# re-ovo/wgpu-path-tracing

Measured on AMD Instinct MI355X. Metric: Msamples/s (rays x bounces / s), higher is better.
Workload: dtype f32

## Files before the change

### wgpu-path-tracing_amd/csrc/pt_device.h

```cpp
#pragma once
#include <hip/hip_runtime.h>
#include <stdint.h>
#include <initializer_list>
#include <variant>
#include "ptmi_layout.h"
#include "ptmi.h"

#define PT_HD __host__ __device__ inline

#define PT_REF_LEAF      0x80000000u
#define PT_REF_NONE      0xFFFFFFFFu
#define PT_LEAF_MAX_TRIS 32u
#define PT_LEAF_OFF_BITS 26u
#define PT_LEAF_OFF_MASK ((1u << PT_LEAF_OFF_BITS) - 1u)

struct DevEnv {
    const float4 *tab;
    const uint2 *alias;
    uint32_t w, h;
    uint32_t sampled;
    float intensity, rotation;
};

struct DevMedium {
// ... 136 lines not shown
              "ptmi_reproject zeroes the four with one memset, ptmi_reproject_status reads them with one copy");
static_assert(kCtRpMoved == kCtRpSamples + 1 && kCtRpMovedCarried == kCtRpMoved + 1,
              "the two motion words follow the four: the same memset zeroes all six, ptmi_motion_status reads the two with one copy");

struct ShadeParams {
    uint32_t bounce, max_bounces, do_mis;
    uint32_t *counts;
    uint32_t emit_records;
    const uint32_t *pid;
};

enum { PT_VARIANT_GLOBAL = 1, PT_VARIANT_LDS = 2, PT_VARIANT_LDS_NODES = 3,
       PT_VARIANT_OWN_LDS = 4, PT_VARIANT_OWN_LDS_NODES = 5, PT_VARIANT_OWN_QLDS = 6, PT_VARIANT_OWN_QLDS_NODES = 7,
       PT_VARIANT_OWN_QGLOBAL = 8, PT_VARIANT_OWN_GLOBAL = 9,
       PT_VARIANT_OWN_LDS16_NODES = 10,
       PT_VARIANT_OWN_QLDS16_NODES = 11,
       PT_VARIANT_COUNT };

enum PtNodes {
    PT_NODES_EXACT,
    PT_NODES_QUANT,
    PT_NODES_EXACT16,
    PT_NODES_QUANT16 };
enum PtWhere {
    PT_LDS_ALL,
    PT_LDS_NODES,
    PT_FROM_MEMORY };
enum PtStack {
    PT_STACK_DEPTH,
    PT_STACK_NODES,
    PT_STACK_SPILL,
    PT_STACK_16BIT,
    PT_STACK_16BIT_SPILL };
struct PtVariant { PtNodes nodes; PtWhere where; PtStack stack; bool own; };
constexpr PtVariant kPtVariants[PT_VARIANT_COUNT] = {
    {},
    {PT_NODES_EXACT,   PT_FROM_MEMORY, PT_STACK_SPILL,       false},
    {PT_NODES_EXACT,   PT_LDS_ALL,     PT_STACK_DEPTH,       false},
    {PT_NODES_EXACT,   PT_LDS_NODES,   PT_STACK_NODES,       false},
    {PT_NODES_EXACT,   PT_LDS_ALL,     PT_STACK_DEPTH,       true},
    {PT_NODES_EXACT,   PT_LDS_NODES,   PT_STACK_NODES,       true},
    {PT_NODES_QUANT,   PT_LDS_ALL,     PT_STACK_DEPTH,       true},
    {PT_NODES_QUANT,   PT_LDS_NODES,   PT_STACK_NODES,       true},
    {PT_NODES_QUANT,   PT_FROM_MEMORY, PT_STACK_SPILL,       true},
    {PT_NODES_EXACT,   PT_FROM_MEMORY, PT_STACK_SPILL,       true},
    {PT_NODES_EXACT16, PT_LDS_NODES,   PT_STACK_16BIT,       true},
    {PT_NODES_QUANT16, PT_LDS_NODES,   PT_STACK_16BIT_SPILL, true},
};
inline const PtVariant &pt_variant(int v) { return kPtVariants[v > 0 && v < PT_VARIANT_COUNT ? v : 0]; }
inline bool pt_quantised(const PtVariant &r) { return r.nodes == PT_NODES_QUANT || r.nodes == PT_NODES_QUANT16; }
inline bool pt_spills(const PtVariant &r, int wgs) {
    return r.stack == PT_STACK_SPILL || r.stack == PT_STACK_16BIT_SPILL || (r.stack == PT_STACK_NODES && wgs == 1);
}
inline size_t pt_lds_bytes(const PtVariant &r, uint32_t n_nodes, uint32_t n_tris, int entries) {
    if (r.where == PT_FROM_MEMORY) return 0;
    const bool narrow = r.nodes == PT_NODES_EXACT16 || r.nodes == PT_NODES_QUANT16;
    return (size_t)n_nodes * (pt_quantised(r) ? 32 : 64) + (r.where == PT_LDS_ALL ? (size_t)n_tris * 48 : 0) +
           (size_t)entries * 1024 * (narrow ? sizeof(uint16_t) : sizeof(uint32_t));
}

struct TraverseConfig {
    int variant;
    int stack_entries;
    int cull;
    int wgs_per_cu;
    size_t lds_bytes;
    uint32_t *spill;
    int wants_spill;
    int quantized;
};
inline uint32_t pt_variant_code(const TraverseConfig &cfg) { return (uint32_t)cfg.variant * 10u + (uint32_t)cfg.wgs_per_cu; }
#ifndef PT_QCACHE_NODES
#define PT_QCACHE_NODES 256
#endif
#define PT_SPILL_ENTRIES 64
size_t pt_spill_bytes(int blocks);

struct DensePixels {
    DevBand band; uint32_t frame0;
    __device__ uint32_t entries() const { return band.rows * band.width; }
    __device__ uint32_t pixel(uint32_t j) const { return j; }
    __device__ uint32_t first_frame(size_t) const { return frame0; }
    __device__ void count_paths(uint32_t) const {}
};
struct ListedPixels {
    DevBand band; const uint32_t *list, *n_active; const float4 *mom;
    unsigned long long *traced;
    __device__ uint32_t entries() const { return *n_active; }
    __device__ uint32_t pixel(uint32_t j) const { return list[j]; }
    __device__ uint32_t first_frame(size_t oi) const { return (uint32_t)mom[oi].z; }
    __device__ void count_paths(uint32_t paths) const { atomicAdd(traced, (unsigned long long)paths); }
};
struct BakedPixels {
    DevBand band; const uint32_t *covered; uint32_t n, frame0;
    __device__ uint32_t entries() const { return n; }
    __device__ uint32_t pixel(uint32_t j) const { return covered[j]; }
    __device__ uint32_t first_frame(size_t) const { return frame0; }
    __device__ void count_paths(uint32_t) const {}
};
using DevPixels = std::variant<DensePixels, ListedPixels, BakedPixels>;
struct CameraSource { const ptmi_camera *cam; uint32_t proj; };
struct BakeSurface { const float4 *texels; float bias; };
struct ProbeSet { const float4 *probes; uint32_t shift, cols, count; };
using DevRays = std::variant<CameraSource, BakeSurface, ProbeSet>;
void pt_launch_raygen(hipStream_t s, int blocks, const DevRays &rays, const DevPixels &px, uint32_t n_frames, DevPaths p, uint32_t *count_out);
void pt_launch_raygen_list(hipStream_t s, const DevRays &rays, uint32_t width, uint32_t n, const uint32_t *xs, const uint32_t *ys,
                           const uint32_t *frames, DevPaths p);
float4 *pt_launch_bake_dilate(hipStream_t s, uint32_t W, uint32_t H, uint32_t passes, const float4 *texels, const float4 *out,
                              float4 *a, float4 *b);
struct DevProbeAtlas { const float4 *out; const float4 *probes; uint32_t W, shift, cols, count; };
// ... 108 lines not shown
```

### wgpu-path-tracing_amd/csrc/traverse.hip

```cpp
#include "pt_device.h"
#include "pt_math.h"
#include "traverse_common.h"

namespace {

struct GlobalMem {
    glb_f4p wn, tp;
    PT_DEV void node(uint32_t i, bool, Boxes &o) const { float4 a, b, c, r; load_node(wn + 4u * (size_t)i, a, b, c, r); boxes_of(a, b, c, r, o); }
    PT_DEV bool open(uint32_t ref, bool, v3, v3, float, uint32_t &first, uint32_t &cnt, uint32_t &cursor) const {
        open_plain(ref, first, cnt, cursor); return true;
    }
    PT_DEV void tri(uint32_t cursor, uint32_t k, bool, float4 &a, float4 &b, float4 &c) const {
        glb_f4p p = tp + 3u * (size_t)(cursor + k);
        a = as_f4(p[0]); b = as_f4(p[1]); c = as_f4(p[2]);
    }
};
template <bool TRIS_IN_LDS>
struct LdsMem {
    lds_f4p wn, tl; glb_f4p tg;
    PT_DEV void node(uint32_t i, bool, Boxes &o) const {
        lds_f4p p = wn + 4u * i;
        boxes_of(as_f4(p[0]), as_f4(p[1]), as_f4(p[2]), as_f4(p[3]), o);
    }
    PT_DEV bool open(uint32_t ref, bool, v3, v3, float, uint32_t &first, uint32_t &cnt, uint32_t &cursor) const {
        open_plain(ref, first, cnt, cursor); return true;
    }
    PT_DEV void tri(uint32_t cursor, uint32_t k, bool, float4 &a, float4 &b, float4 &c) const {
        const uint32_t i = cursor + k;
        if (TRIS_IN_LDS) { lds_f4p p = tl + 3u * i; a = as_f4(p[0]); b = as_f4(p[1]); c = as_f4(p[2]); }
        else { glb_f4p p = tg + 3u * (size_t)i; a = as_f4(p[0]); b = as_f4(p[1]); c = as_f4(p[2]); }
    }
};

typedef const __attribute__((address_space(1))) uint32_t *glb_u32p;
typedef uint32_t u4v __attribute__((ext_vector_type(4)));
typedef const __attribute__((address_space(1))) u4v *glb_u4p;
typedef const __attribute__((address_space(3))) u4v *lds_u4p;
struct QuantMem {
    glb_u4p qn; glb_u32p ls; glb_f4p tp;
    float ox, oy, oz, sx, sy, sz;
    lds_u4p qc; uint32_t n_cached;
    PT_DEV void node(uint32_t i, bool, Boxes &b) const {
        u4v l, r;
        if (i < n_cached) { l = qc[2u * i]; r = qc[2u * i + 1u]; }
        else { l = qn[2u * (size_t)i]; r = qn[2u * (size_t)i + 1u]; }
        b.lx0 = fma1(sx, (float)(l.x & 0xFFFFu), ox); b.ly0 = fma1(sy, (float)(l.x >> 16), oy);
        b.lz0 = fma1(sz, (float)(l.y & 0xFFFFu), oz); b.lx1 = fma1(sx, (float)(l.y >> 16), ox);
        b.ly1 = fma1(sy, (float)(l.z & 0xFFFFu), oy); b.lz1 = fma1(sz, (float)(l.z >> 16), oz);
        b.rx0 = fma1(sx, (float)(r.x & 0xFFFFu), ox); b.ry0 = fma1(sy, (float)(r.x >> 16), oy);
        b.rz0 = fma1(sz, (float)(r.y & 0xFFFFu), oz); b.rx1 = fma1(sx, (float)(r.y >> 16), ox);
        b.ry1 = fma1(sy, (float)(r.z & 0xFFFFu), oy); b.rz1 = fma1(sz, (float)(r.z >> 16), oz);
        b.lref = l.w; b.rref = r.w;
    }
    PT_DEV bool open(uint32_t ref, bool plain, v3 o, v3 inv, float limit, uint32_t &first, uint32_t &cnt, uint32_t &cursor) const {
        if (plain) { open_plain(ref, first, cnt, cursor); return true; }
        const uint32_t off = ref & ~PT_REF_LEAF;
        glb_u32p h = ls + off;
        const float lx = __uint_as_float(h[0]), ly = __uint_as_float(h[1]), lz = __uint_as_float(h[2]);
        first = h[3];
        const float hx = __uint_as_float(h[4]), hy = __uint_as_float(h[5]), hz = __uint_as_float(h[6]);
        cnt = h[7];
        cursor = off + 8u;
        float tl;
        const bool pass = slab(lx, ly, lz, hx, hy, hz, o, inv, tl);
        return pass & !(tl > limit);
    }
    PT_DEV void tri(uint32_t cursor, uint32_t k, bool plain, float4 &a, float4 &b, float4 &c) const {
        if (plain) {
            glb_f4p p = tp + 3u * (size_t)(cursor + k);
            a = as_f4(p[0]); b = as_f4(p[1]); c = as_f4(p[2]);
        } else {
            glb_u32p p = ls + cursor + 9u * k;
            a = make_float4(__uint_as_float(p[0]), __uint_as_float(p[1]), __uint_as_float(p[2]), 0.0f);
            b = make_float4(__uint_as_float(p[3]), __uint_as_float(p[4]), __uint_as_float(p[5]), 0.0f);
            c = make_float4(__uint_as_float(p[6]), __uint_as_float(p[7]), __uint_as_float(p[8]), 0.0f);
// ... 149 lines not shown
                    cn = cn & (cur != PT_REF_NONE) & ((int)room2(lp, sp, stride) | (int)(SPILL && (sp != bot) & room2(lp, bot, stride)));
                    if (popc(ballot(cn)) * NODE_KEEP < popc(bn)) break;
                }
            }
        }
        };
        if (ballot(slow & active) != 0ull) streams(std::true_type{});
        else streams(std::false_type{});
        const bool stuck = active & !can_node & !can_tri & ((bn | bt) == 0ull);
        const bool done = active & (occluded | stuck | ((cur == PT_REF_NONE) & (lp == top)));
        if (done) { io.finish(slot, best, occluded); active = false; cur = PT_REF_NONE; lp = top; }
    }
#ifdef PT_UTIL_STATS
    if (lane == 0u) for (int i = 0; i < 8; i++) atomicAdd(&g_util[MODE][i], (unsigned long long)ut[i]);
    for (int i = 8; i < 10; i++) if (ut[i]) atomicAdd(&g_util[MODE][i], (unsigned long long)ut[i]);
#endif
}

constexpr int GBLOCK = 256;

template <int MODE, bool CULL, int STACK, bool QUANT, class IO>
__global__ __launch_bounds__(GBLOCK) void k_trace_global(DevScene sc, IO io, const uint32_t *__restrict__ count_ptr,
                                                         uint32_t *__restrict__ spill) {
    __shared__ uint32_t stk[STACK * GBLOCK];
    const uint32_t count = *count_ptr;
    const uint32_t gw = (threadIdx.x >> 6) * gridDim.x + blockIdx.x;
    uint32_t *sp = spill + (size_t)blockIdx.x * GBLOCK + threadIdx.x;
    if constexpr (QUANT) {
        __shared__ uint4 qcache[2 * PT_QCACHE_NODES];
        const uint32_t nc = sc.q_cached < PT_QCACHE_NODES ? sc.q_cached : PT_QCACHE_NODES;
        if (blockIdx.x * 64u >= count) return;
        for (uint32_t i = threadIdx.x; i < 2u * nc; i += GBLOCK) qcache[i] = sc.qnodes[i];
        __syncthreads();
        if (gw * 64u >= count) return;
        QuantMem m{(glb_u4p)sc.qnodes, (glb_u32p)sc.leaf_stream, (glb_f4p)sc.tripos,
                   sc.q_origin[0], sc.q_origin[1], sc.q_origin[2], sc.q_scale[0], sc.q_scale[1], sc.q_scale[2],
                   (lds_u4p)qcache, nc};
        trace_wave<MODE, CULL, STACK, true, PT_REFILL_GLOBAL>(m, sc, io, count, gw, gridDim.x * (GBLOCK / 64), stk + threadIdx.x, GBLOCK, sp, gridDim.x * GBLOCK);
    } else {
        if (gw * 64u >= count) return;
        GlobalMem m{(glb_f4p)sc.wnodes, (glb_f4p)sc.tripos};
        trace_wave<MODE, CULL, STACK, true, PT_REFILL_GLOBAL>(m, sc, io, count, gw, gridDim.x * (GBLOCK / 64), stk + threadIdx.x, GBLOCK, sp, gridDim.x * GBLOCK);
    }
}

constexpr int LBLOCK = 1024;

template <int MODE, bool CULL, int STACK, bool TRIS_IN_LDS, bool SPILL, class IO>
__global__ __launch_bounds__(LBLOCK) void k_trace_lds(DevScene sc, IO io, const uint32_t *__restrict__ count_ptr,
                                                      uint32_t *__restrict__ spill) {
    extern __shared__ float4 smem[];
    const uint32_t count = *count_ptr;
    if (blockIdx.x * 64u >= count) return;
    const uint32_t nw = 4u * sc.n_wnodes, nt = TRIS_IN_LDS ? 3u * sc.n_tris : 0u;
    for (uint32_t i = threadIdx.x; i < nw; i += LBLOCK) smem[i] = sc.wnodes[i];
    for (uint32_t i = threadIdx.x; i < nt; i += LBLOCK) smem[nw + i] = sc.tripos[i];
    __syncthreads();
    const uint32_t gw = (threadIdx.x >> 6) * gridDim.x + blockIdx.x;
    if (gw * 64u >= count) return;
    LdsMem<TRIS_IN_LDS> m{(lds_f4p)smem, (lds_f4p)(smem + nw), (glb_f4p)sc.tripos};
    uint32_t *stk = reinterpret_cast<uint32_t *>(smem + nw + nt) + threadIdx.x;
    trace_wave<MODE, CULL, STACK, SPILL, REFILL_AT>(m, sc, io, count, gw, gridDim.x * (LBLOCK / 64), stk, LBLOCK,
                                           SPILL ? spill + (size_t)blockIdx.x * LBLOCK + threadIdx.x : nullptr, gridDim.x * LBLOCK);
}

template <int MODE, bool CULL, int STACK, bool TRIS, bool SPILL, class IO>
void launch_lds(hipStream_t s, int wgs, const TraverseConfig &cfg, const DevScene &sc, const IO &io, const uint32_t *count) {
    allow_all_lds<k_trace_lds<MODE, CULL, STACK, TRIS, SPILL, IO>>();
    hipLaunchKernelGGL((k_trace_lds<MODE, CULL, STACK, TRIS, SPILL, IO>), dim3(wgs), dim3(LBLOCK), cfg.lds_bytes, s, sc, io, count,
                       SPILL ? cfg.spill : nullptr);
}
template <int MODE, bool CULL, bool QUANT, class IO>
void launch_global(hipStream_t s, int cus, const DevScene &sc, const IO &io, const uint32_t *count, uint32_t *spill) {
    const int per_cu = resident_wgs_per_cu<k_trace_global<MODE, CULL, 16, QUANT, IO>>(GBLOCK);
    hipLaunchKernelGGL((k_trace_global<MODE, CULL, 16, QUANT, IO>), dim3(per_cu * cus), dim3(GBLOCK), 0, s, sc, io, count, spill);
}

template <int MODE, bool CULL, class IO>
void launch(hipStream_t s, int blocks, const TraverseConfig &cfg, const DevScene &sc, const IO &io, const uint32_t *count) {
    const int cus = blocks / 8 > 0 ? blocks / 8 : 1;
    const int wgs = cfg.wgs_per_cu * cus;
    if (cfg.variant == PT_VARIANT_LDS_NODES && cfg.wgs_per_cu == 1) {
        launch_lds<MODE, CULL, 16, false, true>(s, wgs, cfg, sc, io, count);
    } else if (cfg.variant == PT_VARIANT_LDS_NODES) {
        if (cfg.stack_entries <= 15) launch_lds<MODE, CULL, 15, false, false>(s, wgs, cfg, sc, io, count);
        else launch_lds<MODE, CULL, 16, false, false>(s, wgs, cfg, sc, io, count);
    } else if (cfg.variant == PT_VARIANT_LDS) {
        if (cfg.stack_entries <= 16) launch_lds<MODE, CULL, 16, true, false>(s, cus, cfg, sc, io, count);
        else launch_lds<MODE, CULL, 32, true, false>(s, cus, cfg, sc, io, count);
    } else if (cfg.quantized && sc.qnodes) {
        launch_global<MODE, CULL, true>(s, cus, sc, io, count, cfg.spill);
    } else {
        launch_global<MODE, CULL, false>(s, cus, sc, io, count, cfg.spill);
    }
}

}

void pt_launch_extend(hipStream_t s, int blocks, const TraverseConfig &cfg, const DevScene &sc, DevPaths p,
                      const uint32_t *queue, const uint32_t *count, float2 *hits) {
    launch_extend_io(cfg, p, queue, hits, [&](auto mode, auto cull, const auto &io) {
        launch<decltype(mode)::value, decltype(cull)::value>(s, blocks, cfg, sc, io, count);
    });
}

void pt_launch_shadow(hipStream_t s, int blocks, const TraverseConfig &cfg, const DevScene &sc, DevPaths p,
                      DevShadow sh, const uint32_t *shadow_queue, const uint32_t *count, uint8_t *occ) {
    launch_shadow_io(cfg, p, sh, shadow_queue, occ, [&](auto mode, auto cull, const auto &io) {
        launch<decltype(mode)::value, decltype(cull)::value>(s, blocks, cfg, sc, io, count);
    });
}

size_t pt_spill_bytes(int blocks) {
// ... 16 lines not shown
```

### wgpu-path-tracing_amd/csrc/traverse_common.h

```cpp
#pragma once
#include "pt_device.h"
#include "pt_math.h"
#include <atomic>
#include <type_traits>

namespace {

constexpr int MODE_EXTEND = 0, MODE_SHADOW = 1;
#ifndef PT_REFILL_AT
#define PT_REFILL_AT 36
#endif
constexpr int REFILL_AT = PT_REFILL_AT;
#ifndef PT_REFILL_GLOBAL
#define PT_REFILL_GLOBAL 52
#endif
#ifndef PT_NODE_STEPS
#define PT_NODE_STEPS 8
#endif
#ifndef PT_LEAF_STEPS
#define PT_LEAF_STEPS 4
#endif
#ifndef PT_LEAF_KEEP
#define PT_LEAF_KEEP 3
#endif
constexpr int NODE_STEPS = PT_NODE_STEPS, LEAF_STEPS = PT_LEAF_STEPS, LEAF_KEEP = PT_LEAF_KEEP;
#ifndef PT_SPILL_NODE_UNROLL
#define PT_SPILL_NODE_UNROLL 8
#endif

typedef float f4v __attribute__((ext_vector_type(4)));
typedef const __attribute__((address_space(3))) f4v *lds_f4p;
typedef const __attribute__((address_space(1))) f4v *glb_f4p;
typedef __attribute__((address_space(3))) uint32_t *lds_u32p;
PT_DEV uint32_t uniform(uint32_t v) { return (uint32_t)__builtin_amdgcn_readfirstlane((int)v); }
PT_DEV uint64_t ballot(bool p) { return __builtin_amdgcn_ballot_w64(p); }
PT_DEV int popc(uint64_t m) { return __builtin_popcount((uint32_t)m) + __builtin_popcount((uint32_t)(m >> 32)); }
PT_DEV bool room2(lds_u32p lp, lds_u32p sp, int stride) {
    return (int)((uint32_t)(uintptr_t)lp - (uint32_t)(uintptr_t)sp) >= stride * 4;
}
PT_DEV float4 as_f4(f4v v) { return make_float4(v.x, v.y, v.z, v.w); }
PT_DEV void load_node(glb_f4p p, float4 &a, float4 &b, float4 &c, float4 &d) {
    a = as_f4(p[0]); b = as_f4(p[1]); c = as_f4(p[2]); d = as_f4(p[3]);
}

struct Boxes { float lx0, ly0, lz0, lx1, ly1, lz1, rx0, ry0, rz0, rx1, ry1, rz1; uint32_t lref, rref; };
PT_DEV void boxes_of(float4 a, float4 b, float4 c, float4 r, Boxes &o) {
    o.lx0 = a.x; o.ly0 = a.y; o.lz0 = a.z; o.lx1 = a.w; o.ly1 = b.x; o.lz1 = b.y;
    o.rx0 = b.z; o.ry0 = b.w; o.rz0 = c.x; o.rx1 = c.y; o.ry1 = c.z; o.rz1 = c.w;
    o.lref = __float_as_uint(r.x); o.rref = __float_as_uint(r.y);
}
PT_DEV void open_plain(uint32_t ref, uint32_t &first, uint32_t &cnt, uint32_t &cursor) {
    first = ref & PT_LEAF_OFF_MASK; cnt = ((ref >> PT_LEAF_OFF_BITS) & (PT_LEAF_MAX_TRIS - 1u)) + 1u; cursor = first;
}

#ifdef PT_UTIL_STATS
static __device__ unsigned long long g_util[2][16];
#define UTIL(i, v) (ut[i] += (uint32_t)(v))
#else
#define UTIL(i, v) ((void)0)
#endif

PT_DEV bool slab(float bx0, float by0, float bz0, float bx1, float by1, float bz1, v3 o, v3 inv, float &tmin) {
    float t1x = (bx0 - o.x) * inv.x, t2x = (bx1 - o.x) * inv.x;
    float t1y = (by0 - o.y) * inv.y, t2y = (by1 - o.y) * inv.y;
    float t1z = (bz0 - o.z) * inv.z, t2z = (bz1 - o.z) * inv.z;
    tmin = max1(max1(min1(t1x, t2x), min1(t1y, t2y)), min1(t1z, t2z));
    float tmax = min1(min1(max1(t1x, t2x), max1(t1y, t2y)), max1(t1z, t2z));
    return tmax >= tmin && tmax >= 0.0f;
}

PT_DEV float cull_limit(float t) { return fma1(t, 1.001f, 1e-4f); }

struct Hit { float t; uint32_t tri; };

PT_DEV float2 pack_hit(const Hit &h) {
    if (h.tri == PT_REF_NONE) return make_float2(-1.0f, __uint_as_float(PT_REF_NONE));
    return make_float2(h.t, __uint_as_float(h.tri));
}

struct ExtendIO {
    const float4 *O, *D; const uint32_t *queue; float2 *hits;
    PT_DEV bool fetch(uint32_t slot, v3 &o, v3 &d, float &tlim) const {
        uint32_t p = queue ? queue[slot] : slot;
        float4 o4 = O[p], d4 = D[p];
        o = xyz(o4); d = xyz(d4); tlim = 0.0f;
        return true;
    }
    PT_DEV void finish(uint32_t slot, const Hit &h, bool) const { st_stream(&hits[slot], pack_hit(h)); }
    PT_DEV bool fetch(uint32_t slot, v3 &o, v3 &d, float &tlim, uint32_t &) const { return fetch(slot, o, d, tlim); }
    PT_DEV void finish(uint32_t slot, const Hit &h, bool occ, uint32_t) const { finish(slot, h, occ); }
};
struct ShadowIO {
    float *L; const float4 *rec; const uint32_t *sq; uint32_t l_stride, cap;
    PT_DEV bool fetch(uint32_t &slot, v3 &o, v3 &d, float &tlim) const {
        uint32_t i = sq ? sq[slot] : slot;
// ... 79 lines not shown
```

### wgpu-path-tracing_amd/csrc/traverse_own.hip

```cpp
#include "pt_device.h"
#include "pt_math.h"
#include "traverse_common.h"

namespace {

#ifndef PT_OWN_REFILL_AT
#define PT_OWN_REFILL_AT 44
#endif

typedef const __attribute__((address_space(1))) uint32_t *glb_u32p;
typedef uint32_t u4v __attribute__((ext_vector_type(4)));
typedef const __attribute__((address_space(1))) u4v *glb_u4p;
typedef const __attribute__((address_space(3))) u4v *lds_u4p;

PT_DEV bool slab_fma(float bx0, float by0, float bz0, float bx1, float by1, float bz1, v3 inv, v3 n, float &tmin) {
    const float t1x = fma1(bx0, inv.x, n.x), t2x = fma1(bx1, inv.x, n.x);
    const float t1y = fma1(by0, inv.y, n.y), t2y = fma1(by1, inv.y, n.y);
    const float t1z = fma1(bz0, inv.z, n.z), t2z = fma1(bz1, inv.z, n.z);
    tmin = max1(max1(min1(t1x, t2x), min1(t1y, t2y)), min1(t1z, t2z));
    const float tmax = min1(min1(max1(t1x, t2x), max1(t1y, t2y)), max1(t1z, t2z));
    return tmax >= tmin && tmax >= 0.0f;
}
PT_DEV bool slab_t(float t1x, float t2x, float t1y, float t2y, float t1z, float t2z, float &tmin) {
    tmin = max1(max1(min1(t1x, t2x), min1(t1y, t2y)), min1(t1z, t2z));
    const float tmax = min1(min1(max1(t1x, t2x), max1(t1y, t2y)), max1(t1z, t2z));
    return tmax >= tmin && tmax >= 0.0f;
}
PT_DEV v3 rcp3(v3 d) { return mk3(rcp1(d.x), rcp1(d.y), rcp1(d.z)); }

template <bool TRIS_IN_LDS>
struct OwnLdsMem {
    lds_f4p wn, tl; glb_f4p tg;
    struct Pre { v3 inv, n; };
    PT_DEV Pre prep(v3 o, v3 inv) const { return Pre{inv, mk3(-(o.x * inv.x), -(o.y * inv.y), -(o.z * inv.z))}; }
    PT_DEV v3 inv_of(const Pre &p, v3) const { return p.inv; }
    PT_DEV void test(uint32_t i, const Pre &p, float &tl_, float &tr_, bool &hl, bool &hr, uint32_t &lref, uint32_t &rref) const {
        lds_f4p q = wn + 4u * i;
        const float4 a = as_f4(q[0]), b = as_f4(q[1]), c = as_f4(q[2]), r = as_f4(q[3]);
        hl = slab_fma(a.x, a.y, a.z, a.w, b.x, b.y, p.inv, p.n, tl_);
        hr = slab_fma(b.z, b.w, c.x, c.y, c.z, c.w, p.inv, p.n, tr_);
        lref = __float_as_uint(r.x); rref = __float_as_uint(r.y);
    }
    PT_DEV void tri(uint32_t i, float4 &a, float4 &b, float4 &c) const {
        if (TRIS_IN_LDS) { lds_f4p p = tl + 3u * i; a = as_f4(p[0]); b = as_f4(p[1]); c = as_f4(p[2]); }
        else { glb_f4p p = tg + 3u * (size_t)i; a = as_f4(p[0]); b = as_f4(p[1]); c = as_f4(p[2]); }
    }
};
struct OwnGlobalMem {
    glb_f4p wn, tg;
    struct Pre { v3 inv, n; };
    PT_DEV Pre prep(v3 o, v3 inv) const { return Pre{inv, mk3(-(o.x * inv.x), -(o.y * inv.y), -(o.z * inv.z))}; }
    PT_DEV v3 inv_of(const Pre &p, v3) const { return p.inv; }
    PT_DEV void test(uint32_t i, const Pre &p, float &tl_, float &tr_, bool &hl, bool &hr, uint32_t &lref, uint32_t &rref) const {
        float4 a, b, c, r; load_node(wn + 4u * (size_t)i, a, b, c, r);
        hl = slab_fma(a.x, a.y, a.z, a.w, b.x, b.y, p.inv, p.n, tl_);
        hr = slab_fma(b.z, b.w, c.x, c.y, c.z, c.w, p.inv, p.n, tr_);
        lref = __float_as_uint(r.x); rref = __float_as_uint(r.y);
    }
    PT_DEV void tri(uint32_t i, float4 &a, float4 &b, float4 &c) const {
        glb_f4p p = tg + 3u * (size_t)i; a = as_f4(p[0]); b = as_f4(p[1]); c = as_f4(p[2]);
    }
};
template <bool ALL_IN_LDS, bool TRIS_IN_LDS>
struct OwnQuantMem {
    lds_u4p qc; glb_u4p qn; uint32_t n_cached; lds_f4p tl; glb_f4p tg;
    float ox, oy, oz, sx, sy, sz;
    struct Pre { v3 s, o; };
    PT_DEV Pre prep(v3 o, v3 inv) const {
        const v3 n = mk3(-(o.x * inv.x), -(o.y * inv.y), -(o.z * inv.z));
        return Pre{mk3(sx * inv.x, sy * inv.y, sz * inv.z), mk3(fma1(ox, inv.x, n.x), fma1(oy, inv.y, n.y), fma1(oz, inv.z, n.z))};
    }
    PT_DEV v3 inv_of(const Pre &, v3 d) const { return rcp3(d); }
    PT_DEV void test(uint32_t i, const Pre &p, float &tl_, float &tr_, bool &hl, bool &hr, uint32_t &lref, uint32_t &rref) const {
        u4v l, r;
        if (ALL_IN_LDS || i < n_cached) { l = qc[2u * i]; r = qc[2u * i + 1u]; }
        else { l = qn[2u * (size_t)i]; r = qn[2u * (size_t)i + 1u]; }
        hl = slab_t(fma1((float)(l.x & 0xFFFFu), p.s.x, p.o.x), fma1((float)(l.y >> 16), p.s.x, p.o.x),
                    fma1((float)(l.x >> 16), p.s.y, p.o.y), fma1((float)(l.z & 0xFFFFu), p.s.y, p.o.y),
                    fma1((float)(l.y & 0xFFFFu), p.s.z, p.o.z), fma1((float)(l.z >> 16), p.s.z, p.o.z), tl_);
        hr = slab_t(fma1((float)(r.x & 0xFFFFu), p.s.x, p.o.x), fma1((float)(r.y >> 16), p.s.x, p.o.x),
                    fma1((float)(r.x >> 16), p.s.y, p.o.y), fma1((float)(r.z & 0xFFFFu), p.s.y, p.o.y),
                    fma1((float)(r.y & 0xFFFFu), p.s.z, p.o.z), fma1((float)(r.z >> 16), p.s.z, p.o.z), tr_);
        lref = l.w; rref = r.w;
    }
    PT_DEV void tri(uint32_t i, float4 &a, float4 &b, float4 &c) const {
        if (TRIS_IN_LDS) { lds_f4p p = tl + 3u * i; a = as_f4(p[0]); b = as_f4(p[1]); c = as_f4(p[2]); }
        else { glb_f4p p = tg + 3u * (size_t)i; a = as_f4(p[0]); b = as_f4(p[1]); c = as_f4(p[2]); }
    }
};

template <int MODE, bool CULL, int STACK, bool SPILL, bool FROM_MEMORY, class Mem, class IO, class E>
// ... 195 lines not shown
                    if (hr & rl) { *lp = (E)rref; lp -= stride; }
                    const bool il = hl & !ll, ir = hr & !rl;
                    const bool left_first = tl <= tr;
                    if (il & ir) { *sp = (E)(left_first ? rref : lref); sp += stride; cur = left_first ? lref : rref; }
                    else if (il) cur = lref;
                    else if (ir) cur = rref;
                    else if (sp != bot) { sp -= stride; cur = *sp; }
                    else if (SPILL && spn != 0u) {
                        const int fit = (int)((uint32_t)(uintptr_t)lp - (uint32_t)(uintptr_t)bot) / (stride * (int)sizeof(E));
                        uint32_t n = spn < 8u ? spn : 8u;
                        n = (int)n < fit ? n : (fit > 1 ? (uint32_t)fit : 1u);
                        spn -= n;
                        for (uint32_t j = 0; j + 1u < n; j++) { *sp = (E)spill[(size_t)(spn + j) * spill_lanes]; sp += stride; }
                        cur = spill[(size_t)(spn + n - 1u) * spill_lanes];
                    }
                    else cur = PT_REF_NONE;
                }
                if (rep + 1 < NODE_STEPS) {
                    cn = cn & (cur != PT_REF_NONE) & ((int)room(lp, sp, stride) | (int)(SPILL && (sp != bot) & room(lp, bot, stride)));
                    uint64_t rm = ballot(room(lp, sp, stride));
                    if (SPILL) rm |= ballot(sp != bot) & ballot(room(lp, bot, stride));
                    cnm = cnm & ballot(cur != PT_REF_NONE) & rm;
                    if (popc(cnm) * NODE_KEEP < popc(bn)) break;
                }
            }
        }
        };
        if (ballot(slow & active) != 0ull) streams(std::true_type{});
        else streams(std::false_type{});
        const bool stuck = active & !can_node & !can_tri & ((bn | bt) == 0ull);
        const bool done = active & (occluded | stuck | ((cur == PT_REF_NONE) & (lp == top)));
        if (done) {
            active = false; cur = PT_REF_NONE; lp = top;
            fin = true; fin_occ = occluded;
            if (stuck) { slow = true; n_redo++; }
        }
    }
    if (n_redo) atomicAdd(sc.verify_stat, (unsigned long long)n_redo);
#ifdef PT_UTIL_STATS
    if (lane == 0u) for (int i = 0; i < 8; i++) atomicAdd(&g_util[MODE][i], (unsigned long long)ut[i]);
    for (int i = 8; i < 10; i++) if (ut[i]) atomicAdd(&g_util[MODE][i], (unsigned long long)ut[i]);
#endif
}

constexpr int GBLOCK = 256, LBLOCK = 1024;

template <int MODE, bool CULL, int STACK, int LAYOUT, bool TRIS, bool SPILL, class IO>
__global__ __launch_bounds__(LBLOCK) __attribute__((amdgpu_waves_per_eu((STACK == 15 || LAYOUT == 3) ? 8 : 4))) void k_own_lds(const DevScene *__restrict__ scp, IO io, const uint32_t *__restrict__ count_ptr,
                                                                    uint32_t *__restrict__ spill, int nstack) {
    const DevScene &sc = *scp;
    extern __shared__ float4 smem[];
    const uint32_t count = *count_ptr;
    if (blockIdx.x * 64u >= count) return;
    const uint32_t nw = ((LAYOUT == 1 || LAYOUT == 3) ? 2u : 4u) * sc.n_wnodes, nt = TRIS ? 3u * sc.n_own_tris : 0u;
    const float4 *src = LAYOUT == 1 ? reinterpret_cast<const float4 *>(sc.qnodes) : LAYOUT == 3 ? reinterpret_cast<const float4 *>(sc.qnodes16)
                      : LAYOUT == 2 ? sc.wnodes16 : sc.wnodes;
    for (uint32_t i = threadIdx.x; i < nw; i += LBLOCK) smem[i] = src[i];
    for (uint32_t i = threadIdx.x; i < nt; i += LBLOCK) smem[nw + i] = sc.tripos[i];
    __syncthreads();
    const uint32_t gw = (threadIdx.x >> 6) * gridDim.x + blockIdx.x;
    if (gw * 64u >= count) return;
    uint32_t *stk = reinterpret_cast<uint32_t *>(smem + nw + nt) + threadIdx.x;
    uint32_t *sp = SPILL ? spill + (size_t)blockIdx.x * LBLOCK + threadIdx.x : nullptr;
    if constexpr (LAYOUT == 2) {
        OwnLdsMem<TRIS> m{(lds_f4p)smem, (lds_f4p)(smem + nw), (glb_f4p)sc.tripos};
        uint16_t *stk16 = reinterpret_cast<uint16_t *>(smem + nw + nt) + threadIdx.x;
        trace_wave_own<MODE, CULL, STACK, false, false>(m, sc, io, count, gw, gridDim.x * (LBLOCK / 64), stk16, LBLOCK);
    } else if constexpr (LAYOUT == 3) {
        OwnQuantMem<true, false> m{(lds_u4p)smem, (glb_u4p)sc.qnodes16, sc.n_wnodes, (lds_f4p)nullptr, (glb_f4p)sc.tripos,
                                   sc.q_origin[0], sc.q_origin[1], sc.q_origin[2], sc.q_scale[0], sc.q_scale[1], sc.q_scale[2]};
        uint16_t *stk16 = reinterpret_cast<uint16_t *>(smem + nw + nt) + threadIdx.x;
        trace_wave_own<MODE, CULL, 0, true, false>(m, sc, io, count, gw, gridDim.x * (LBLOCK / 64), stk16, LBLOCK, sp, gridDim.x * LBLOCK, nstack);
    } else if constexpr (LAYOUT == 1) {
        OwnQuantMem<true, TRIS> m{(lds_u4p)smem, (glb_u4p)sc.qnodes, sc.n_wnodes, (lds_f4p)(smem + nw), (glb_f4p)sc.tripos,
                                  sc.q_origin[0], sc.q_origin[1], sc.q_origin[2], sc.q_scale[0], sc.q_scale[1], sc.q_scale[2]};
        trace_wave_own<MODE, CULL, STACK, SPILL, false>(m, sc, io, count, gw, gridDim.x * (LBLOCK / 64), stk, LBLOCK, sp, gridDim.x * LBLOCK);
    } else {
        OwnLdsMem<TRIS> m{(lds_f4p)smem, (lds_f4p)(smem + nw), (glb_f4p)sc.tripos};
        trace_wave_own<MODE, CULL, STACK, SPILL, false>(m, sc, io, count, gw, gridDim.x * (LBLOCK / 64), stk, LBLOCK, sp, gridDim.x * LBLOCK);
    }
}

template <int MODE, bool CULL, int STACK, int LAYOUT, bool TRIS, bool SPILL, class IO>
void launch_own_lds(hipStream_t s, int cus, const TraverseConfig &cfg, const DevScene *sc, const IO &io, const uint32_t *count) {
    allow_all_lds<k_own_lds<MODE, CULL, STACK, LAYOUT, TRIS, SPILL, IO>>();
    hipLaunchKernelGGL((k_own_lds<MODE, CULL, STACK, LAYOUT, TRIS, SPILL, IO>), dim3(cfg.wgs_per_cu * cus), dim3(LBLOCK), cfg.lds_bytes, s,
                       sc, io, count, SPILL ? cfg.spill : nullptr, STACK ? 0 : cfg.stack_entries);
}

template <int MODE, bool CULL, bool QUANT, class IO>
__global__ __launch_bounds__(GBLOCK) void k_own_global(const DevScene *__restrict__ scp, IO io, const uint32_t *__restrict__ count_ptr, uint32_t *__restrict__ spill) {
    const DevScene &sc = *scp;
    __shared__ uint32_t stk[16 * GBLOCK];
    const uint32_t count = *count_ptr;
    const uint32_t gw = (threadIdx.x >> 6) * gridDim.x + blockIdx.x;
    uint32_t *sp = spill + (size_t)blockIdx.x * GBLOCK + threadIdx.x;
    if constexpr (QUANT) {
        __shared__ uint4 qcache[2 * PT_QCACHE_NODES];
        const uint32_t nc = sc.q_cached < PT_QCACHE_NODES ? sc.q_cached : PT_QCACHE_NODES;
        if (blockIdx.x * 64u >= count) return;
        for (uint32_t i = threadIdx.x; i < 2u * nc; i += GBLOCK) qcache[i] = sc.qnodes[i];
        __syncthreads();
        if (gw * 64u >= count) return;
        OwnQuantMem<false, false> m{(lds_u4p)qcache, (glb_u4p)sc.qnodes, nc, (lds_f4p)nullptr, (glb_f4p)sc.tripos,
                                    sc.q_origin[0], sc.q_origin[1], sc.q_origin[2], sc.q_scale[0], sc.q_scale[1], sc.q_scale[2]};
        trace_wave_own<MODE, CULL, 16, true, true>(m, sc, io, count, gw, gridDim.x * (GBLOCK / 64), stk + threadIdx.x, GBLOCK, sp, gridDim.x * GBLOCK);
    } else {
        if (gw * 64u >= count) return;
        OwnGlobalMem m{(glb_f4p)sc.wnodes, (glb_f4p)sc.tripos};
        trace_wave_own<MODE, CULL, 16, true, true>(m, sc, io, count, gw, gridDim.x * (GBLOCK / 64), stk + threadIdx.x, GBLOCK, sp, gridDim.x * GBLOCK);
    }
}
template <int MODE, bool CULL, bool QUANT, class IO>
void launch_own_global(hipStream_t s, int cus, const DevScene *sc, const IO &io, const uint32_t *count, uint32_t *spill) {
    const int per_cu = resident_wgs_per_cu<k_own_global<MODE, CULL, QUANT, IO>>(GBLOCK);
    hipLaunchKernelGGL((k_own_global<MODE, CULL, QUANT, IO>), dim3(per_cu * cus), dim3(GBLOCK), 0, s, sc, io, count, spill);
}

template <int MODE, bool CULL, class IO>
void launch_own(hipStream_t s, int blocks, const TraverseConfig &cfg, const DevScene &hsc, const IO &io, const uint32_t *count) {
    const int cus = blocks / 8 > 0 ? blocks / 8 : 1;
    const DevScene *sc = hsc.self;
    const bool two = cfg.wgs_per_cu == 2;
    switch (cfg.variant) {
    case PT_VARIANT_OWN_LDS:
        if (cfg.stack_entries <= 16) launch_own_lds<MODE, CULL, 16, 0, true, false>(s, cus, cfg, sc, io, count);
        else launch_own_lds<MODE, CULL, 32, 0, true, false>(s, cus, cfg, sc, io, count);
        break;
    case PT_VARIANT_OWN_LDS_NODES:
        if (two) launch_own_lds<MODE, CULL, 15, 0, false, false>(s, cus, cfg, sc, io, count);
        else launch_own_lds<MODE, CULL, 16, 0, false, true>(s, cus, cfg, sc, io, count);
// ... 44 lines not shown
```

### wgpu-path-tracing_amd/csrc/traverse_pick.hip

```cpp
#include "ptmi_ctx.h"

#include <algorithm>
#include <cstdlib>
#include <iterator>
#include <utility>

namespace {

constexpr size_t kLdsMax = 160 * 1024;

size_t lds_scene_bytes(const ptmi_ctx *c) { return (size_t)c->img.n_wnodes * 64 + (size_t)c->img.n_tris * 48; }

bool size_variant(const ptmi_ctx *c, int variant, int wgs, TraverseConfig &cfg) {
    const PtVariant &r = pt_variant(variant);
    const uint32_t depth = std::max(c->img.depth, c->img.ref_depth);
    int entries = 0;
    bool ok = true;
    switch (r.stack) {
    case PT_STACK_DEPTH: entries = depth + 2 <= 16 ? 16 : depth + 2 <= 32 ? 32 : 0; ok = wgs == 1 && entries != 0; break;
    case PT_STACK_NODES: entries = wgs == 2 ? 15 : 16; ok = wgs == 1 || (wgs == 2 && depth + 1 <= 15); break;
    case PT_STACK_SPILL: entries = 16; ok = wgs == 1; break;
    case PT_STACK_16BIT: entries = 15; ok = wgs == 2 && depth + 1 <= 15; break;
    case PT_STACK_16BIT_SPILL: {
        const size_t nq = (size_t)c->sc.n_wnodes * 32;
        entries = (c->sc.qnodes16 && nq + 64 < kLdsMax / 2) ? std::min<int>(15, (int)((kLdsMax / 2 - 64 - nq) / 2048)) : 0;
        if (const char *e = std::getenv("PTMI_OWN_Q16_ENTRIES"))
            entries = std::min(entries, std::max(8, std::atoi(e)));
        ok = wgs == 2 && entries >= 8;
        break;
    }
    }
    ok = ok && (!pt_quantised(r) || (c->sc.own && c->img.quantised)) && (r.nodes != PT_NODES_EXACT16 || c->sc.wnodes16 != nullptr);
    cfg.variant = variant; cfg.wgs_per_cu = wgs; cfg.stack_entries = entries;
    cfg.wants_spill = pt_spills(r, wgs) ? 1 : 0;
    cfg.quantized = pt_quantised(r) ? 1 : 0;
    cfg.lds_bytes = pt_lds_bytes(r, c->sc.n_wnodes, c->sc.own ? c->sc.n_own_tris : c->sc.n_tris, entries);
    return ok && cfg.lds_bytes <= kLdsMax / (size_t)wgs;
}

TraverseConfig traverse_config(const ptmi_ctx *c, bool closest_hit) {
    const bool own = c->sc.own, big = lds_scene_bytes(c) > ((size_t)4 << 20);
    const int traversal = c->opt.traversal;
    TraverseConfig cfg{};
    cfg.cull = c->opt.cull ? 1 : 0;
    auto pick = [&](int variant, int wgs) { return size_variant(c, variant, wgs, cfg); };
    const bool mem_quant = traversal == PTMI_TRAVERSAL_GLOBAL || (traversal == PTMI_TRAVERSAL_AUTO && big);
    auto from_memory = [&]() {
        if (!own) { pick(PT_VARIANT_GLOBAL, 1); cfg.quantized = mem_quant; cfg.wgs_per_cu = 2; }
        else pick(c->img.quantised && mem_quant ? PT_VARIANT_OWN_QGLOBAL : PT_VARIANT_OWN_GLOBAL, 1);
        return cfg;
    };
    if (traversal == PTMI_TRAVERSAL_GLOBAL || traversal == PTMI_TRAVERSAL_GLOBAL_EXACT) return from_memory();
    if (own && traversal == PTMI_TRAVERSAL_AUTO)
        if (const char *e = std::getenv(closest_hit ? "PTMI_OWN_EXTEND" : "PTMI_OWN_SHADOW")) {
            int code = std::atoi(e);
            if (code < 40) code = code == 20 ? 102 : code == 21 ? 112 : (code % 10) * 10 + (code >= 10 ? 2 : 1);
            if (pt_variant(code / 10).own && pick(code / 10, code % 10)) return cfg;
        }
    struct Pick { int variant, wgs; };
    static const Pick own_auto[] = {{PT_VARIANT_OWN_LDS_NODES, 2}, {PT_VARIANT_OWN_LDS16_NODES, 2}, {PT_VARIANT_OWN_QLDS_NODES, 2},
                                    {PT_VARIANT_OWN_QLDS16_NODES, 2}, {PT_VARIANT_OWN_LDS, 1}, {PT_VARIANT_OWN_QLDS, 1},
                                    {PT_VARIANT_OWN_QLDS_NODES, 1}, {PT_VARIANT_OWN_LDS_NODES, 1}};
    static const Pick own_lds[] = {{PT_VARIANT_OWN_LDS, 1}, {PT_VARIANT_OWN_QLDS, 1}};
    static const Pick ref_closest[] = {{PT_VARIANT_LDS_NODES, 2}, {PT_VARIANT_LDS, 1}, {PT_VARIANT_LDS_NODES, 1}};
    static const Pick ref_lds[] = {{PT_VARIANT_LDS, 1}};
    auto all = [](const auto &l) { return std::make_pair(std::begin(l), std::end(l)); };
    const auto picks = traversal == PTMI_TRAVERSAL_LDS ? (own ? all(own_lds) : all(ref_lds))
                     : own ? (big ? std::make_pair(own_auto, own_auto) : all(own_auto)) : closest_hit ? all(ref_closest) : all(ref_lds);
    if (own || c->sc.root_ref != PT_REF_NONE)
        for (const Pick *p = picks.first; p != picks.second; p++)
            if (pick(p->variant, p->wgs)) {
                if (p->variant == PT_VARIANT_LDS) cfg.wgs_per_cu = 2;
                return cfg;
            }
    return from_memory();
}

}

PT_HOST {

bool walks_memory_quantised(const TraverseConfig &cfg) {
    return cfg.quantized && pt_variant(cfg.variant).where == PT_FROM_MEMORY;
}

int traverse_pick(const ptmi_ctx *c, bool closest_hit, TraverseConfig &cfg) {
    cfg = traverse_config(c, closest_hit);
    if (closest_hit && c->opt.traversal == PTMI_TRAVERSAL_LDS && pt_variant(cfg.variant).where != PT_LDS_ALL)
        return fail(c, PTMI_E_UNSUPPORTED, "scene needs %zu B of LDS plus the stack; it does not fit in %zu B", lds_scene_bytes(c), kLdsMax);
    return PTMI_OK;
// ... 27 lines not shown
```

Measured before the change: 12260.

## Store LDS BVH nodes in planar quad layout with fixed plane stride

Changes the LDS node storage from interleaved 64-byte nodes (4 consecutive float4) to a planar layout where each of the four float4 quads of a node lives in its own plane with a fixed stride, for exact/16-bit node variants using the node-only stack at 2 WGs per CU. The intent is to cut LDS bank conflicts when lanes of a wave read different nodes, since each quad read then touches consecutive addresses across nodes. Staging now scatters into the planes, and the LDS budget is reserved at a fixed plane size, which may reject scenes whose node count exceeds the plane and changes which variant gets picked.

```diff
diff --git a/wgpu-path-tracing_amd/csrc/pt_device.h b/wgpu-path-tracing_amd/csrc/pt_device.h
--- a/wgpu-path-tracing_amd/csrc/pt_device.h
+++ b/wgpu-path-tracing_amd/csrc/pt_device.h
@@ -212,10 +212,17 @@
 inline bool pt_spills(const PtVariant &r, int wgs) {
     return r.stack == PT_STACK_SPILL || r.stack == PT_STACK_16BIT_SPILL || (r.stack == PT_STACK_NODES && wgs == 1);
 }
-inline size_t pt_lds_bytes(const PtVariant &r, uint32_t n_nodes, uint32_t n_tris, int entries) {
+#define PT_NODE_PLANE_EXACT   ((80u * 1024u - 15u * 1024u * 4u) / 64u)
+#define PT_NODE_PLANE_EXACT16 ((80u * 1024u - 15u * 1024u * 2u) / 64u)
+inline uint32_t pt_node_plane_stride(const PtVariant &r, int wgs, uint32_t n_nodes) {
+    if (r.nodes == PT_NODES_EXACT16) return PT_NODE_PLANE_EXACT16;
+    if (r.nodes == PT_NODES_EXACT && r.stack == PT_STACK_NODES && wgs == 2) return PT_NODE_PLANE_EXACT;
+    return n_nodes;
+}
+inline size_t pt_lds_bytes(const PtVariant &r, int wgs, uint32_t n_nodes, uint32_t n_tris, int entries) {
     if (r.where == PT_FROM_MEMORY) return 0;
     const bool narrow = r.nodes == PT_NODES_EXACT16 || r.nodes == PT_NODES_QUANT16;
-    return (size_t)n_nodes * (pt_quantised(r) ? 32 : 64) + (r.where == PT_LDS_ALL ? (size_t)n_tris * 48 : 0) +
+    return (size_t)pt_node_plane_stride(r, wgs, n_nodes) * (pt_quantised(r) ? 32 : 64) + (r.where == PT_LDS_ALL ? (size_t)n_tris * 48 : 0) +
            (size_t)entries * 1024 * (narrow ? sizeof(uint16_t) : sizeof(uint32_t));
 }
 
diff --git a/wgpu-path-tracing_amd/csrc/traverse.hip b/wgpu-path-tracing_amd/csrc/traverse.hip
--- a/wgpu-path-tracing_amd/csrc/traverse.hip
+++ b/wgpu-path-tracing_amd/csrc/traverse.hip
@@ -15,12 +15,12 @@
         a = as_f4(p[0]); b = as_f4(p[1]); c = as_f4(p[2]);
     }
 };
-template <bool TRIS_IN_LDS>
+template <bool TRIS_IN_LDS, uint32_t PLANE>
 struct LdsMem {
     lds_f4p wn, tl; glb_f4p tg;
     PT_DEV void node(uint32_t i, bool, Boxes &o) const {
-        lds_f4p p = wn + 4u * i;
-        boxes_of(as_f4(p[0]), as_f4(p[1]), as_f4(p[2]), as_f4(p[3]), o);
+        boxes_of(as_f4(wn[node_quad<PLANE>(i, 0)]), as_f4(wn[node_quad<PLANE>(i, 1)]), as_f4(wn[node_quad<PLANE>(i, 2)]),
+                 as_f4(wn[node_quad<PLANE>(i, 3)]), o);
     }
     PT_DEV bool open(uint32_t ref, bool, v3, v3, float, uint32_t &first, uint32_t &cnt, uint32_t &cursor) const {
         open_plain(ref, first, cnt, cursor); return true;
@@ -276,13 +276,14 @@
     extern __shared__ float4 smem[];
     const uint32_t count = *count_ptr;
     if (blockIdx.x * 64u >= count) return;
-    const uint32_t nw = 4u * sc.n_wnodes, nt = TRIS_IN_LDS ? 3u * sc.n_tris : 0u;
-    for (uint32_t i = threadIdx.x; i < nw; i += LBLOCK) smem[i] = sc.wnodes[i];
+    constexpr uint32_t PLANE = STACK == 15 ? PT_NODE_PLANE_EXACT : 0u;
+    const uint32_t nw = 4u * (PLANE ? PLANE : sc.n_wnodes), nt = TRIS_IN_LDS ? 3u * sc.n_tris : 0u;
+    stage_nodes<PLANE>(smem, sc.wnodes, sc.n_wnodes, threadIdx.x, LBLOCK);
     for (uint32_t i = threadIdx.x; i < nt; i += LBLOCK) smem[nw + i] = sc.tripos[i];
     __syncthreads();
     const uint32_t gw = (threadIdx.x >> 6) * gridDim.x + blockIdx.x;
     if (gw * 64u >= count) return;
-    LdsMem<TRIS_IN_LDS> m{(lds_f4p)smem, (lds_f4p)(smem + nw), (glb_f4p)sc.tripos};
+    LdsMem<TRIS_IN_LDS, PLANE> m{(lds_f4p)smem, (lds_f4p)(smem + nw), (glb_f4p)sc.tripos};
     uint32_t *stk = reinterpret_cast<uint32_t *>(smem + nw + nt) + threadIdx.x;
     trace_wave<MODE, CULL, STACK, SPILL, REFILL_AT>(m, sc, io, count, gw, gridDim.x * (LBLOCK / 64), stk, LBLOCK,
                                            SPILL ? spill + (size_t)blockIdx.x * LBLOCK + threadIdx.x : nullptr, gridDim.x * LBLOCK);
diff --git a/wgpu-path-tracing_amd/csrc/traverse_common.h b/wgpu-path-tracing_amd/csrc/traverse_common.h
--- a/wgpu-path-tracing_amd/csrc/traverse_common.h
+++ b/wgpu-path-tracing_amd/csrc/traverse_common.h
@@ -41,6 +41,13 @@
 PT_DEV float4 as_f4(f4v v) { return make_float4(v.x, v.y, v.z, v.w); }
 PT_DEV void load_node(glb_f4p p, float4 &a, float4 &b, float4 &c, float4 &d) {
     a = as_f4(p[0]); b = as_f4(p[1]); c = as_f4(p[2]); d = as_f4(p[3]);
+}
+
+template <uint32_t PLANE>
+PT_DEV uint32_t node_quad(uint32_t i, uint32_t k) { return PLANE ? k * PLANE + i : 4u * i + k; }
+template <uint32_t PLANE>
+PT_DEV void stage_nodes(float4 *smem, const float4 *src, uint32_t n_nodes, uint32_t tid, uint32_t threads) {
+    for (uint32_t j = tid; j < 4u * n_nodes; j += threads) smem[node_quad<PLANE>(j / 4u, j % 4u)] = src[j];
 }
 
 struct Boxes { float lx0, ly0, lz0, lx1, ly1, lz1, rx0, ry0, rz0, rx1, ry1, rz1; uint32_t lref, rref; };
diff --git a/wgpu-path-tracing_amd/csrc/traverse_own.hip b/wgpu-path-tracing_amd/csrc/traverse_own.hip
--- a/wgpu-path-tracing_amd/csrc/traverse_own.hip
+++ b/wgpu-path-tracing_amd/csrc/traverse_own.hip
@@ -28,15 +28,15 @@
 }
 PT_DEV v3 rcp3(v3 d) { return mk3(rcp1(d.x), rcp1(d.y), rcp1(d.z)); }
 
-template <bool TRIS_IN_LDS>
+template <bool TRIS_IN_LDS, uint32_t PLANE>
 struct OwnLdsMem {
     lds_f4p wn, tl; glb_f4p tg;
     struct Pre { v3 inv, n; };
     PT_DEV Pre prep(v3 o, v3 inv) const { return Pre{inv, mk3(-(o.x * inv.x), -(o.y * inv.y), -(o.z * inv.z))}; }
     PT_DEV v3 inv_of(const Pre &p, v3) const { return p.inv; }
     PT_DEV void test(uint32_t i, const Pre &p, float &tl_, float &tr_, bool &hl, bool &hr, uint32_t &lref, uint32_t &rref) const {
-        lds_f4p q = wn + 4u * i;
-        const float4 a = as_f4(q[0]), b = as_f4(q[1]), c = as_f4(q[2]), r = as_f4(q[3]);
+        const float4 a = as_f4(wn[node_quad<PLANE>(i, 0)]), b = as_f4(wn[node_quad<PLANE>(i, 1)]), c = as_f4(wn[node_quad<PLANE>(i, 2)]),
+                     r = as_f4(wn[node_quad<PLANE>(i, 3)]);
         hl = slab_fma(a.x, a.y, a.z, a.w, b.x, b.y, p.inv, p.n, tl_);
         hr = slab_fma(b.z, b.w, c.x, c.y, c.z, c.w, p.inv, p.n, tr_);
         lref = __float_as_uint(r.x); rref = __float_as_uint(r.y);
@@ -338,10 +338,13 @@
     extern __shared__ float4 smem[];
     const uint32_t count = *count_ptr;
     if (blockIdx.x * 64u >= count) return;
-    const uint32_t nw = ((LAYOUT == 1 || LAYOUT == 3) ? 2u : 4u) * sc.n_wnodes, nt = TRIS ? 3u * sc.n_own_tris : 0u;
+    constexpr uint32_t QUADS = (LAYOUT == 1 || LAYOUT == 3) ? 2u : 4u;
+    constexpr uint32_t PLANE = LAYOUT == 2 ? PT_NODE_PLANE_EXACT16 : (LAYOUT == 0 && STACK == 15) ? PT_NODE_PLANE_EXACT : 0u;
+    const uint32_t nw = QUADS * (PLANE ? PLANE : sc.n_wnodes), nt = TRIS ? 3u * sc.n_own_tris : 0u;
     const float4 *src = LAYOUT == 1 ? reinterpret_cast<const float4 *>(sc.qnodes) : LAYOUT == 3 ? reinterpret_cast<const float4 *>(sc.qnodes16)
                       : LAYOUT == 2 ? sc.wnodes16 : sc.wnodes;
-    for (uint32_t i = threadIdx.x; i < nw; i += LBLOCK) smem[i] = src[i];
+    if constexpr (PLANE != 0u) stage_nodes<PLANE>(smem, src, sc.n_wnodes, threadIdx.x, LBLOCK);
+    else for (uint32_t i = threadIdx.x; i < nw; i += LBLOCK) smem[i] = src[i];
     for (uint32_t i = threadIdx.x; i < nt; i += LBLOCK) smem[nw + i] = sc.tripos[i];
     __syncthreads();
     const uint32_t gw = (threadIdx.x >> 6) * gridDim.x + blockIdx.x;
@@ -349,7 +352,7 @@
     uint32_t *stk = reinterpret_cast<uint32_t *>(smem + nw + nt) + threadIdx.x;
     uint32_t *sp = SPILL ? spill + (size_t)blockIdx.x * LBLOCK + threadIdx.x : nullptr;
     if constexpr (LAYOUT == 2) {
-        OwnLdsMem<TRIS> m{(lds_f4p)smem, (lds_f4p)(smem + nw), (glb_f4p)sc.tripos};
+        OwnLdsMem<TRIS, PLANE> m{(lds_f4p)smem, (lds_f4p)(smem + nw), (glb_f4p)sc.tripos};
         uint16_t *stk16 = reinterpret_cast<uint16_t *>(smem + nw + nt) + threadIdx.x;
         trace_wave_own<MODE, CULL, STACK, false, false>(m, sc, io, count, gw, gridDim.x * (LBLOCK / 64), stk16, LBLOCK);
     } else if constexpr (LAYOUT == 3) {
@@ -362,7 +365,7 @@
                                   sc.q_origin[0], sc.q_origin[1], sc.q_origin[2], sc.q_scale[0], sc.q_scale[1], sc.q_scale[2]};
         trace_wave_own<MODE, CULL, STACK, SPILL, false>(m, sc, io, count, gw, gridDim.x * (LBLOCK / 64), stk, LBLOCK, sp, gridDim.x * LBLOCK);
     } else {
-        OwnLdsMem<TRIS> m{(lds_f4p)smem, (lds_f4p)(smem + nw), (glb_f4p)sc.tripos};
+        OwnLdsMem<TRIS, PLANE> m{(lds_f4p)smem, (lds_f4p)(smem + nw), (glb_f4p)sc.tripos};
         trace_wave_own<MODE, CULL, STACK, SPILL, false>(m, sc, io, count, gw, gridDim.x * (LBLOCK / 64), stk, LBLOCK, sp, gridDim.x * LBLOCK);
     }
 }
diff --git a/wgpu-path-tracing_amd/csrc/traverse_pick.hip b/wgpu-path-tracing_amd/csrc/traverse_pick.hip
--- a/wgpu-path-tracing_amd/csrc/traverse_pick.hip
+++ b/wgpu-path-tracing_amd/csrc/traverse_pick.hip
@@ -34,8 +34,8 @@
     cfg.variant = variant; cfg.wgs_per_cu = wgs; cfg.stack_entries = entries;
     cfg.wants_spill = pt_spills(r, wgs) ? 1 : 0;
     cfg.quantized = pt_quantised(r) ? 1 : 0;
-    cfg.lds_bytes = pt_lds_bytes(r, c->sc.n_wnodes, c->sc.own ? c->sc.n_own_tris : c->sc.n_tris, entries);
-    return ok && cfg.lds_bytes <= kLdsMax / (size_t)wgs;
+    cfg.lds_bytes = pt_lds_bytes(r, wgs, c->sc.n_wnodes, c->sc.own ? c->sc.n_own_tris : c->sc.n_tris, entries);
+    return ok && c->sc.n_wnodes <= pt_node_plane_stride(r, wgs, c->sc.n_wnodes) && cfg.lds_bytes <= kLdsMax / (size_t)wgs;
 }
 
 TraverseConfig traverse_config(const ptmi_ctx *c, bool closest_hit) {
```

New measurement: 12060. 1.6% lower.
